# rom1504/clip-retrieval

Hardware: AMD Instinct MI355X
Metric: images/sec embedded (ViT-L/14 bs=256; each sample = image + caption through both towers) (higher is better)
Workload: dtype bf16

## Files before the change

### clip-retrieval_amd/csrc/clip_kernels.hip

```cpp

#include <hip/hip_runtime.h>
#include <stdint.h>
#include <stdlib.h>
#include <math.h>
#include "clip_kernels.h"
#include "gemm_common.h"

namespace clipx {

constexpr int G_TM = 128, G_TN = 128, G_BK = 64;
constexpr int G_STAGE_BYTES = (G_TM + G_TN) * G_BK * 2;
constexpr int G_GROUP_M = 8;

template <int EPI, bool GLDS, bool DEEP = false, bool F16 = false>
__global__ __launch_bounds__(256, (DEEP && !CLIPX_MFMA16) ? 1 : 2) void gemm_bf16_kernel(const bf16* __restrict__ A, const bf16* __restrict__ W,
                                                          const float* __restrict__ bias, void* __restrict__ outp,
                                                          const float* __restrict__ table, int T, int M, int N,
                                                          int K, int row0, const float* __restrict__ rowscale,
                                                          bf16* __restrict__ out16, int kz) {
  extern __shared__ __attribute__((aligned(16))) unsigned char smem[];
  const int tid = threadIdx.x;
  const int lane = tid & 63, w = tid >> 6;
  const int wn = w & 1, wm = w >> 1;
  const int hb = lane >> 5, l31 = lane & 31;
// ... 686 lines not shown
  const dim3 grid((M + 3) / 4), block(256);
#define LN_CASE(NV)                                                                                           \
  case NV * 256:                                                                                              \
    if (out_kind == 1) hipLaunchKernelGGL((layernorm_kernel<NV, 1>), grid, block, 0, st, x, gamma, beta, y, M, eps, (bf16*)nullptr); \
    else if (out_kind == 2) hipLaunchKernelGGL((layernorm_kernel<NV, 2>), grid, block, 0, st, x, gamma, beta, y, M, eps, (bf16*)nullptr); \
    else hipLaunchKernelGGL((layernorm_kernel<NV, 0>), grid, block, 0, st, x, gamma, beta, y, M, eps, y16);    \
    break;
  switch (d) {
    LN_CASE(1) LN_CASE(2) LN_CASE(3) LN_CASE(4) LN_CASE(5) LN_CASE(6) LN_CASE(7) LN_CASE(8)
    default: return hipErrorInvalidValue;
  }
#undef LN_CASE
  return hipGetLastError();
}

template <int FMT>
__global__ __launch_bounds__(256) void im2col_kernel(const void* __restrict__ pixels, int B, int S, int P, int Kp,
                                                    float m0, float m1, float m2, float i0, float i1, float i2,
                                                    bf16* __restrict__ out) {
  const int gdim = S / P, T = gdim * gdim + 1, PP = P * P, K = 3 * PP, nch = Kp / 8;
  const int64_t total = (int64_t)B * T * nch;
  for (int64_t idx = (int64_t)blockIdx.x * blockDim.x + threadIdx.x; idx < total; idx += (int64_t)gridDim.x * blockDim.x) {
    const int ch = (int)(idx % nch);
    const int64_t row = idx / nch;
    const int t = (int)(row % T), b = (int)(row / T);
    bf16x8 o;
    const int tp = t > 0 ? t - 1 : 0;
    const int py = tp / gdim, px = tp - py * gdim;
    float raw[8];
    int cc[8];
#pragma unroll
    for (int e = 0; e < 8; ++e) {
      const int k = ch * 8 + e;
      const int kk = k < K ? k : K - 1;
      const int c = kk / PP, rem = kk - c * PP;
      const int iy = rem / P, ix = rem - iy * P;
      const int yy = py * P + iy, xx = px * P + ix;
      cc[e] = c;
      if (FMT == 0) raw[e] = reinterpret_cast<const float*>(pixels)[(((size_t)b * 3 + c) * S + yy) * S + xx];
      else raw[e] = (float)reinterpret_cast<const unsigned char*>(pixels)[(((size_t)b * S + yy) * S + xx) * 3 + c];
    }
#pragma unroll
    for (int e = 0; e < 8; ++e) {
      float v = raw[e];
      if (FMT != 0) {
        const int c = cc[e];
        const float mean = c == 0 ? m0 : (c == 1 ? m1 : m2), sd = c == 0 ? i0 : (c == 1 ? i1 : i2);
        v = __fdiv_rn(__fsub_rn(__fdiv_rn(v, 255.f), mean), sd);
      }
      o[e] = (t > 0 && ch * 8 + e < K) ? (bf16)v : (bf16)0.f;
    }
    *reinterpret_cast<bf16x8*>(out + (size_t)row * Kp + ch * 8) = o;
  }
}

hipError_t launch_im2col(const void* pixels, int fmt, int B, int S, int P, int Kp, const float* mean,
                         const float* stdv, bf16* out, hipStream_t st) {
  if (B <= 0) return hipSuccess;
  const int gdim = S / P, T = gdim * gdim + 1;
  const int64_t total = (int64_t)B * T * (Kp / 8);
  const int blocks = (int)((total + 255) / 256 < 65536 * 4 ? (total + 255) / 256 : 65536 * 4);
  if (fmt == 0)
    hipLaunchKernelGGL(im2col_kernel<0>, dim3(blocks), dim3(256), 0, st, pixels, B, S, P, Kp, 0.f, 0.f, 0.f, 1.f, 1.f, 1.f, out);
  else
    hipLaunchKernelGGL(im2col_kernel<1>, dim3(blocks), dim3(256), 0, st, pixels, B, S, P, Kp, mean[0], mean[1], mean[2],
                       stdv[0], stdv[1], stdv[2], out);
  return hipGetLastError();
}

__device__ __forceinline__ f32x16 attn_mfma(bf16x8 a, bf16x8 b, f32x16 c) {
  return __builtin_amdgcn_mfma_f32_32x32x16_f16(__builtin_bit_cast(f16x8, a), __builtin_bit_cast(f16x8, b), c, 0, 0, 0);
}
__device__ __forceinline__ unsigned attn_pack_p(float p0, float p1) {
  typedef float f32x2_t __attribute__((ext_vector_type(2)));
  typedef _Float16 f16x2_t __attribute__((ext_vector_type(2)));
  return __builtin_bit_cast(unsigned, __builtin_convertvector((f32x2_t){p0, p1}, f16x2_t));
}

__device__ long long g_attn_phase[8192 * 4];
#ifdef CLIPX_ABLATE
__device__ int g_attn_pk_timer = 0;
#endif
template <int DH, int NKB, int NW, int QPW, bool CAUSAL, bool RECOMP, bool TIMER = false>
__global__ __launch_bounds__(NW * 64, (2 * NW + 3) / 4) void attention_kernel(const bf16* __restrict__ qkv, bf16* __restrict__ out, int Tin,
                                                              int H, float scale_log2e, int dbg, int q_blocks,
                                                              const int* __restrict__ offs, const int* __restrict__ lens) {
  constexpr int TP = NKB * 32;
  constexpr int CH = DH / 8;
  constexpr int KS = DH / 16;
  constexpr int KROW = DH == 64 ? 128 : 176;
  constexpr int DV = (DH + 31) / 32 * 32, NB = DV / 32;
  constexpr int VT_STRIDE = TP * 2 + 8;
  extern __shared__ __attribute__((aligned(16))) unsigned char smem[];
  unsigned char* sK = smem;
  unsigned char* sVt = smem + TP * KROW;
  const int tid = threadIdx.x, lane = tid & 63, w = tid >> 6;
  const int hb = lane >> 5, l31 = lane & 31;
  long long tph[4] = {0, 0, 0, 0};
  long long tst = TIMER ? (long long)__builtin_readcyclecounter() : 0;
#define A_STAMP(i) if (TIMER) { const long long n_ = (long long)__builtin_readcyclecounter(); tph[i] += n_ - tst; tst = n_; }
  const int b = blockIdx.x / H, h = blockIdx.x - b * H;
  const int ld = 3 * H * DH;
  const int T = lens ? lens[b] : Tin;
  const size_t row0 = offs ? (size_t)offs[b] : (size_t)b * Tin;
  const bf16* qbase = qkv + row0 * ld + h * DH;
  const bf16* kbase = qbase + H * DH;
  const bf16* vbase = qbase + 2 * H * DH;
  auto kchunk = [](int key, int c) -> int { return DH == 64 ? (c ^ ((key >> 1) & 7)) : c; };

  bf16x8 qf_all[QPW][KS];
#pragma unroll
  for (int qi = 0; qi < QPW; ++qi) {
    const int qpos = (qi * NW + w) * 32 + l31;
    const int qrow = qpos < T ? qpos : T - 1;
#pragma unroll
    for (int s = 0; s < KS; ++s) {
      const uint4 v = *reinterpret_cast<const uint4*>(qbase + (size_t)qrow * ld + 16 * s + 8 * hb);
      qf_all[qi][s] = *reinterpret_cast<const bf16x8*>(&v);
    }
  }

  if (dbg != 2) {
  {
    constexpr int KIT = (TP * CH + NW * 64 - 1) / (NW * 64);
    uint4 kv[KIT];
#pragma unroll
    for (int it = 0; it < KIT; ++it) {
      const int i = tid + it * NW * 64;
      int key = i / CH;
      const int c = i - key * CH;
      key = key < T ? key : T - 1;
      kv[it] = *reinterpret_cast<const uint4*>(kbase + (size_t)key * ld + c * 8);
    }
#pragma unroll
    for (int it = 0; it < KIT; ++it) {
      const int i = tid + it * NW * 64;
      const int key = i / CH, c = i - key * CH;
      if (i < TP * CH) {
        const uint4 v = key < T ? kv[it] : make_uint4(0u, 0u, 0u, 0u);
        *reinterpret_cast<uint4*>(sK + key * KROW + (kchunk(key, c) << 4)) = v;
      }
    }
  }
  {
    constexpr int VIT = ((TP / 2) * CH + NW * 64 - 1) / (NW * 64);
    uint4 v0s[VIT], v1s[VIT];
#pragma unroll
    for (int it = 0; it < VIT; ++it) {
      const int i = tid + it * NW * 64;
      const int kp = i / CH, c = i - kp * CH;
      const int k0 = 2 * kp < T ? 2 * kp : T - 1, k1 = 2 * kp + 1 < T ? 2 * kp + 1 : T - 1;
      v0s[it] = *reinterpret_cast<const uint4*>(vbase + (size_t)k0 * ld + c * 8);
      v1s[it] = *reinterpret_cast<const uint4*>(vbase + (size_t)k1 * ld + c * 8);
    }
#pragma unroll
    for (int it = 0; it < VIT; ++it) {
      const int i = tid + it * NW * 64;
      const int kp = i / CH, c = i - kp * CH;
      if (i < (TP / 2) * CH) {
        const uint4 v0 = 2 * kp < T ? v0s[it] : make_uint4(0u, 0u, 0u, 0u);
        const uint4 v1 = 2 * kp + 1 < T ? v1s[it] : make_uint4(0u, 0u, 0u, 0u);
        const unsigned a0[4] = {v0.x, v0.y, v0.z, v0.w}, a1[4] = {v1.x, v1.y, v1.z, v1.w};
#pragma unroll
        for (int jj = 0; jj < 4; ++jj) {
          const unsigned lo = (a0[jj] & 0xffffu) | (a1[jj] << 16);
          const unsigned hi = (a0[jj] >> 16) | (a1[jj] & 0xffff0000u);
          *reinterpret_cast<unsigned*>(sVt + (8 * c + 2 * jj) * VT_STRIDE + kp * 4) = lo;
          *reinterpret_cast<unsigned*>(sVt + (8 * c + 2 * jj + 1) * VT_STRIDE + kp * 4) = hi;
        }
      }
    }
    if (DV > DH) {
      for (int i = tid; i < (DV - DH) * (TP / 2); i += NW * 64) {
        const int r = i / (TP / 2), kp = i - r * (TP / 2);
        *reinterpret_cast<unsigned*>(sVt + (DH + r) * VT_STRIDE + kp * 4) = 0u;
      }
    }
  }
  }
  __syncthreads();
  A_STAMP(0)
  if (dbg == 1) return;

  const int ksw = (l31 >> 1) & 7;
#pragma unroll
  for (int qi = 0; qi < QPW; ++qi) {
    const int qb = qi * NW + w;
    if (qb >= q_blocks) break;
    const int qpos = qb * 32 + l31;
    bf16x8 qf[KS];
#pragma unroll
    for (int s = 0; s < KS; ++s) qf[s] = qf_all[qi][s];
    auto s_block = [&](int kb) -> f32x16 {
      f32x16 sb;
#pragma unroll
      for (int r = 0; r < 16; ++r) sb[r] = 0.f;
      if (!CAUSAL || kb <= qb) {
#pragma unroll
        for (int s = 0; s < KS; ++s) {
          const int c = 2 * s + hb;
          const bf16x8 kf = *reinterpret_cast<const bf16x8*>(sK + (kb * 32 + l31) * KROW + ((DH == 64 ? (c ^ ksw) : c) << 4));
          sb = attn_mfma(kf, qf[s], sb);
        }
      }
      if (kb == NKB - 1 || CAUSAL) {
#pragma unroll
        for (int r = 0; r < 16; ++r) {
          const int key = kb * 32 + (r & 3) + 8 * (r >> 2) + 4 * hb;
          const bool ok = key < T && (!CAUSAL || key <= qpos);
          sb[r] = ok ? sb[r] : -INFINITY;
        }
      }
      return sb;
    };
    f32x16 sacc[RECOMP ? 1 : NKB];
    float mx = -INFINITY;
#pragma unroll(RECOMP ? 1 : NKB)
    for (int kb = 0; kb < NKB; ++kb) {
      const f32x16 sb = s_block(kb);
      if (!RECOMP) sacc[kb] = sb;
#pragma unroll
      for (int r = 0; r < 16; ++r) mx = fmaxf(mx, sb[r]);
    }
    mx = fmaxf(mx, __shfl_xor(mx, 32));
    if (mx == -INFINITY) mx = 0.f;
    const float nmx = -mx * scale_log2e;
    if (TIMER) { asm volatile("" : "+v"(mx)); A_STAMP(1) }

    typedef float f32x2_t __attribute__((ext_vector_type(2)));
    typedef __bf16 bf16x2_t __attribute__((ext_vector_type(2)));
    f32x2_t sum2 = {0.f, 0.f};
    const int tail_keys = T - (NKB - 1) * 32;
    f32x16 oacc[NB];
#pragma unroll
    for (int nb = 0; nb < NB; ++nb)
#pragma unroll
      for (int r = 0; r < 16; ++r) oacc[nb][r] = 0.f;
#pragma unroll(RECOMP ? 1 : NKB)
    for (int kb = 0; kb < NKB; ++kb) {
      if (CAUSAL && kb > qb) continue;
      bf16x8 pf[2];
      const f32x16 sb = RECOMP ? s_block(kb) : sacc[RECOMP ? 0 : kb];
      unsigned pw[8];
      const bool short_tail = !CAUSAL && kb == NKB - 1 && tail_keys <= 4;
#pragma unroll
      for (int r = 0; r < 16; r += 2) {
        if (short_tail && r >= 4) {
          pw[r >> 1] = 0u;
          continue;
        }
        const f32x2_t e = (f32x2_t){sb[r], sb[r + 1]} * (f32x2_t){scale_log2e, scale_log2e} + (f32x2_t){nmx, nmx};
        const f32x2_t pp = {__builtin_amdgcn_exp2f(e[0]), __builtin_amdgcn_exp2f(e[1])};
        sum2 += pp;
        pw[r >> 1] = attn_pack_p(pp[0], pp[1]);
      }
      {
        const uint4 w0 = make_uint4(pw[0], pw[1], pw[2], pw[3]), w1 = make_uint4(pw[4], pw[5], pw[6], pw[7]);
        pf[0] = *reinterpret_cast<const bf16x8*>(&w0);
        pf[1] = *reinterpret_cast<const bf16x8*>(&w1);
      }
#pragma unroll
      for (int s2 = 0; s2 < 2; ++s2)
#pragma unroll
        for (int nb = 0; nb < NB; ++nb) {
          const unsigned char* vp = sVt + (32 * nb + l31) * VT_STRIDE + (kb * 32 + 16 * s2 + 4 * hb) * 2;
          const uint2 lo = *reinterpret_cast<const uint2*>(vp);
          const uint2 hi = *reinterpret_cast<const uint2*>(vp + 16);
          uint4 vv = make_uint4(lo.x, lo.y, hi.x, hi.y);
          oacc[nb] = attn_mfma(*reinterpret_cast<bf16x8*>(&vv), pf[s2], oacc[nb]);
        }
    }
    float sum = sum2[0] + sum2[1];
    sum += __shfl_xor(sum, 32);
    const float inv = sum > 0.f ? 1.f / sum : 0.f;
    if (TIMER) { asm volatile("" : "+v"(oacc[0]), "+v"(oacc[NB - 1])); A_STAMP(2) }
    if (qpos < T) {
      bf16* orow = out + (row0 + qpos) * (H * DH) + h * DH;
#pragma unroll
      for (int nb = 0; nb < NB; ++nb)
#pragma unroll
        for (int g = 0; g < 4; ++g) {
          if (32 * nb + 8 * g >= DH) continue;
          bf16x4 o;
#pragma unroll
          for (int e = 0; e < 4; ++e) o[e] = (bf16)(oacc[nb][4 * g + e] * inv);
          *reinterpret_cast<bf16x4*>(orow + 32 * nb + 8 * g + 4 * hb) = o;
        }
    }
    A_STAMP(3)
  }
  if (TIMER && lane == 0 && blockIdx.x * NW + w < 8192) {
#pragma unroll
    for (int i = 0; i < 4; ++i) g_attn_phase[(blockIdx.x * NW + w) * 4 + i] = tph[i];
  }
#undef A_STAMP
}

#ifndef CLIPX_ATTN_SPIPE
#define CLIPX_ATTN_SPIPE 1
#endif
#ifndef CLIPX_ATTN_ROLES
#define CLIPX_ATTN_ROLES 1
#endif
template <int NKB, int NWT = 6>
__global__ __launch_bounds__(NWT * 64, 1) void attention_pk_kernel(const bf16* __restrict__ qkv, bf16* __restrict__ out, int T, int H,
                                                                  int nheads, float scale_log2e, int q_blocks) {
  constexpr bool EIGHT = NWT == 8;
  constexpr int DH = 64, KS = 4, NW = NWT, NDW = EIGHT ? 8 : (CLIPX_ATTN_ROLES ? 2 : 3), QPW = (NKB + NW - 1) / NW, TP = NKB * 32,
                KROW = 128, NB = 2;
  static_assert(NWT == 6 || NWT == 8, "6 waves (any T of NKB blocks) or 8 (T = 32 (NKB - 1) + 1)");
  static_assert(!CLIPX_ATTN_ROLES || NKB == 9, "the role table below is the one of 9 query blocks");
  static_assert(!EIGHT || (NKB == NW + 1 && QPW == 2), "eight full query blocks + the one-query block");
  constexpr int KBYTES = TP * KROW, VHALF = TP * 64, BUF = KBYTES + 2 * VHALF;
  constexpr int KDMA = TP * 8 / 64 / NDW, VDMA = 2 * TP * 4 / 64 / NDW;
  static_assert(EIGHT || TP * 8 % (64 * NDW) == 0, "the DMA pieces must divide evenly among the issuing waves");
  constexpr int NPIECE = BUF / 1024, PPW = NPIECE / 8, KPIECE = KBYTES / 1024;
  static_assert(!EIGHT || NPIECE % 8 == 0, "the DMA pieces must divide evenly among the eight waves");
  constexpr int MRG = 68;
  const bool tail_on = EIGHT && q_blocks >= NKB;
  typedef short s16x4 __attribute__((ext_vector_type(4)));
  typedef s16x4 __attribute__((address_space(3))) * lds_s16x4_ptr;
  extern __shared__ __attribute__((aligned(16))) unsigned char smem[];
  const int tid = threadIdx.x, lane = tid & 63;
  const int w = __builtin_amdgcn_readfirstlane(tid >> 6);
  const int hb = lane >> 5, l31 = lane & 31;
  const int ld = 3 * H * DH;
  const unsigned lds_base = __builtin_amdgcn_readfirstlane((unsigned)(uintptr_t)(__attribute__((address_space(3))) unsigned char*)smem);
#ifdef CLIPX_ABLATE
  const bool timer = g_attn_pk_timer != 0;
  long long tph[4] = {0, 0, 0, 0};
  long long tst = timer ? (long long)__builtin_readcyclecounter() : 0;
#define P_STAMP(i) if (timer) { const long long n_ = (long long)__builtin_readcyclecounter(); tph[i] += n_ - tst; tst = n_; }
#else
#define P_STAMP(i)
#endif

  auto blk_of = [&](int qi) -> int {
    if (EIGHT) return qi == 0 ? w : -1;
#if CLIPX_ATTN_ROLES
    if (qi == 0) return w;
    return w == 0 ? 6 : (w == 2 ? 7 : (w == 3 ? 8 : -1));
#else
    return qi * NW + w < NKB ? qi * NW + w : -1;
#endif
  };
#if CLIPX_ATTN_ROLES
  const bool dma_wave = EIGHT || w == 1 || w == 5;
  const int dma_idx = EIGHT ? w : (w == 1 ? 0 : 1);
#else
  const bool dma_wave = EIGHT || w >= NW - NDW;
  const int dma_idx = EIGHT ? w : w - (NW - NDW);
#endif
  float* mrg = reinterpret_cast<float*>(smem + 2 * BUF);

  auto issue = [&](int hd, int buf) {
    if (!dma_wave) return;
    const int ww = dma_idx;
    const int b = hd / H, h = hd - b * H;
    const char* base = reinterpret_cast<const char*>(qkv + (size_t)b * T * ld + h * DH);
    int lane_v = lane;
    asm volatile("" : "+v"(lane_v));
    if constexpr (EIGHT) {
#pragma unroll
      for (int j = 0; j < PPW; ++j) {
        const int piece = ww * PPW + j;
        unsigned off;
        if (piece < KPIECE) {
          const int c = piece * 64 + lane_v;
          const int key = c >> 3, pos = c & 7;
          const int kk = key < T ? key : T - 1;
          off = (unsigned)((kk * ld + H * DH + ((pos ^ ((key >> 1) & 7)) << 3)) * 2);
        } else {
          const int c = (piece - KPIECE) * 64 + lane_v;
          const int nbh = c / (TP * 4), rem = c - nbh * (TP * 4);
          const int key = rem >> 2, pos = rem & 3;
          const int kk = key < T ? key : T - 1;
          off = (unsigned)((kk * ld + 2 * H * DH + 32 * nbh + 8 * pos) * 2);
        }
        const unsigned m0 = lds_base + buf * BUF + piece * 1024;
        asm volatile("s_mov_b32 m0, %2\n\ts_nop 0\n\tglobal_load_lds_dwordx4 %0, %1" ::"v"(off), "s"(base), "s"(m0) : "memory");
      }
      return;
    }
#pragma unroll
    for (int j = 0; j < KDMA; ++j) {
      const int c = (ww * KDMA + j) * 64 + lane_v;
      const int key = c >> 3, pos = c & 7;
      const int kk = key < T ? key : T - 1;
      const unsigned off = (unsigned)((kk * ld + H * DH + ((pos ^ ((key >> 1) & 7)) << 3)) * 2);
      const unsigned m0 = lds_base + buf * BUF + (ww * KDMA + j) * 1024;
      asm volatile("s_mov_b32 m0, %2\n\ts_nop 0\n\tglobal_load_lds_dwordx4 %0, %1" ::"v"(off), "s"(base), "s"(m0) : "memory");
    }
#pragma unroll
    for (int j = 0; j < VDMA; ++j) {
      const int c = (ww * VDMA + j) * 64 + lane_v;
      const int nbh = c / (TP * 4), rem = c - nbh * (TP * 4);
      const int key = rem >> 2, pos = rem & 3;
      const int kk = key < T ? key : T - 1;
      const unsigned off = (unsigned)((kk * ld + 2 * H * DH + 32 * nbh + 8 * pos) * 2);
      const unsigned m0 = lds_base + buf * BUF + KBYTES + (ww * VDMA + j) * 1024;
      asm volatile("s_mov_b32 m0, %2\n\ts_nop 0\n\tglobal_load_lds_dwordx4 %0, %1" ::"v"(off), "s"(base), "s"(m0) : "memory");
    }
  };
  bf16x8 qn[QPW][KS];
  auto load_q = [&](int hd, int qi) {
    const int b = hd / H, h = hd - b * H;
    const bf16* qbase = qkv + (size_t)b * T * ld + h * DH;
    int lane_q = lane;
    asm volatile("" : "+v"(lane_q));
    if (blk_of(qi) < 0) return;
    const int qpos = blk_of(qi) * 32 + (lane_q & 31);
    const int qrow = qpos < T ? qpos : T - 1;
#pragma unroll
    for (int s = 0; s < KS; ++s) {
      const uint4 v = *reinterpret_cast<const uint4*>(qbase + (size_t)qrow * ld + 16 * s + 8 * (lane_q >> 5));
      qn[qi][s] = *reinterpret_cast<const bf16x8*>(&v);
    }
  };

  bf16x8 qt[KS];
  auto load_qt = [&](int hd) {
    const int b = hd / H, h = hd - b * H;
    const bf16* qbase = qkv + (size_t)b * T * ld + h * DH;
    int lane_q = lane;
    asm volatile("" : "+v"(lane_q));
#pragma unroll
    for (int s = 0; s < KS; ++s) {
      const uint4 v = *reinterpret_cast<const uint4*>(qbase + (size_t)(T - 1) * ld + 16 * s + 8 * (lane_q >> 5));
      qt[s] = *reinterpret_cast<const bf16x8*>(&v);
    }
  };
  auto merge_tail = [&](int phd, int par) {
    const float* mt = mrg + par * (NKB * MRG);
    float m = -INFINITY;
#pragma unroll
    for (int j = 0; j < NKB; ++j) m = fmaxf(m, mt[j * MRG]);
    float l = 0.f, o = 0.f;
#pragma unroll
    for (int j = 0; j < NKB; ++j) {
      const float wj = __builtin_amdgcn_exp2f((mt[j * MRG] - m) * scale_log2e);
      l += wj * mt[j * MRG + 1];
      o += wj * mt[j * MRG + 2 + lane];
    }
    const int pb = phd / H, ph = phd - pb * H;
    out[((size_t)pb * T + (T - 1)) * (H * DH) + ph * DH + lane] = (bf16)(l > 0.f ? o / l : 0.f);
  };

  int hd = blockIdx.x;
  if (hd >= nheads) return;
  issue(hd, 0);
#pragma unroll
  for (int qi = 0; qi < QPW; ++qi) load_q(hd, qi);
  if (tail_on) {
    load_qt(hd);
#pragma unroll
    for (int s = 0; s < KS; ++s) asm volatile("" : "+v"(qt[s]));
  }
#pragma unroll
  for (int qi = 0; qi < QPW; ++qi)
#pragma unroll
    for (int s = 0; s < KS; ++s) asm volatile("" : "+v"(qn[qi][s]));
  const int ksw = (l31 >> 1) & 7;
  const unsigned vlane = (unsigned)(((lane & 15) >> 2) * 64 + (16 * ((lane >> 4) & 1)) * 2 + (lane & 3) * 8);
  int buf = 0;
  for (; hd < nheads; hd += gridDim.x, buf ^= 1) {
    if (dma_wave && !(hd != (int)blockIdx.x && w < q_blocks)) asm volatile("s_waitcnt vmcnt(0)" ::: "memory");
    __syncthreads();
    P_STAMP(0)
    const int nxt = hd + gridDim.x;
    if (nxt < nheads) issue(nxt, buf ^ 1);
    P_STAMP(1)
    if (tail_on && w == 0 && hd != (int)blockIdx.x) merge_tail(hd - (int)gridDim.x, buf ^ 1);
    const unsigned char* sK = smem + buf * BUF;
    const unsigned char* sV = sK + KBYTES;
    const int b = hd / H, h = hd - b * H;
#pragma unroll
    for (int qi = 0; qi < QPW; ++qi) {
      const int qb = blk_of(qi);
      if (qb < 0 || qb >= q_blocks) continue;
      const int qpos = qb * 32 + l31;
      bf16x8 qf[KS];
#pragma unroll
      for (int s = 0; s < KS; ++s) qf[s] = qn[qi][s];
      f32x16 sacc[NKB];
      float mx = -INFINITY;
#if CLIPX_ATTN_SPIPE
      {
        typedef int i32x4 __attribute__((ext_vector_type(4)));
        unsigned kaddr[KS];
#pragma unroll
        for (int s = 0; s < KS; ++s) kaddr[s] = lds_base + buf * BUF + l31 * KROW + (((2 * s + hb) ^ ksw) << 4);
        i32x4 KF[2][KS];
#pragma unroll
        for (int s = 0; s < KS; ++s) asm volatile("ds_read_b128 %0, %1" : "=v"(KF[0][s]) : "v"(kaddr[s]));
        __builtin_amdgcn_sched_barrier(0);
#pragma unroll
        for (int kb = 0; kb < NKB; ++kb) {
          asm volatile("s_waitcnt lgkmcnt(0)" ::: "memory");
#pragma unroll
          for (int s = 0; s < KS; ++s) asm volatile("" : "+v"(KF[kb & 1][s]));
          if (kb + 1 < NKB) {
#pragma unroll
            for (int s = 0; s < KS; ++s)
              asm volatile("ds_read_b128 %0, %1 offset:%2" : "=v"(KF[(kb + 1) & 1][s]) : "v"(kaddr[s]), "n"((kb + 1) * 32 * KROW));
          }
          __builtin_amdgcn_sched_barrier(0);
          f32x16 sb;
#pragma unroll
          for (int r = 0; r < 16; ++r) sb[r] = 0.f;
#pragma unroll
          for (int s = 0; s < KS; ++s) sb = attn_mfma(__builtin_bit_cast(bf16x8, KF[kb & 1][s]), qf[s], sb);
          __builtin_amdgcn_sched_barrier(0);
          if (kb > 0) {
#pragma unroll
            for (int r = 0; r < 16; ++r) mx = fmaxf(mx, sacc[kb - 1][r]);
            asm volatile("" : "+v"(mx));
            __builtin_amdgcn_sched_barrier(0);
          }
          if (kb == NKB - 1) {
#pragma unroll
            for (int r = 0; r < 16; ++r) {
              const int key = kb * 32 + (r & 3) + 8 * (r >> 2) + 4 * hb;
              sb[r] = key < T ? sb[r] : -INFINITY;
            }
          }
          sacc[kb] = sb;
        }
#pragma unroll
        for (int r = 0; r < 16; ++r) mx = fmaxf(mx, sacc[NKB - 1][r]);
      }
#else
#pragma unroll
      for (int kb = 0; kb < NKB; ++kb) {
        f32x16 sb;
#pragma unroll
        for (int r = 0; r < 16; ++r) sb[r] = 0.f;
#pragma unroll
        for (int s = 0; s < KS; ++s) {
          const int c = 2 * s + hb;
          const bf16x8 kf = *reinterpret_cast<const bf16x8*>(sK + (kb * 32 + l31) * KROW + ((c ^ ksw) << 4));
          sb = attn_mfma(kf, qf[s], sb);
        }
        if (kb == NKB - 1) {
#pragma unroll
          for (int r = 0; r < 16; ++r) {
            const int key = kb * 32 + (r & 3) + 8 * (r >> 2) + 4 * hb;
            sb[r] = key < T ? sb[r] : -INFINITY;
          }
        }
        sacc[kb] = sb;
#pragma unroll
        for (int r = 0; r < 16; ++r) mx = fmaxf(mx, sb[r]);
      }
#endif
#ifdef CLIPX_ABLATE
      if (timer) { asm volatile("" : "+v"(mx)); P_STAMP(2) }
#endif
#if !CLIPX_ATTN_SPIPE
      if (nxt < nheads) load_q(nxt, qi);
#endif
      mx = fmaxf(mx, __shfl_xor(mx, 32));
      if (mx == -INFINITY) mx = 0.f;
      const float nmx = -mx * scale_log2e;
      typedef float f32x2_t __attribute__((ext_vector_type(2)));
      typedef __bf16 bf16x2_t __attribute__((ext_vector_type(2)));
      f32x2_t sum2 = {0.f, 0.f};
      const int tail_keys = T - (NKB - 1) * 32;
      f32x16 oacc[NB];
#pragma unroll
      for (int nb = 0; nb < NB; ++nb)
#pragma unroll
        for (int r = 0; r < 16; ++r) oacc[nb][r] = 0.f;
#if CLIPX_ATTN_SPIPE
      {
        typedef short s16x8 __attribute__((ext_vector_type(8)));
        unsigned pw[8];
        unsigned pnew[8];
        s16x8 vf[2][NB];
        auto read_v = [&](int kb, int s2) {
#pragma unroll
          for (int nb = 0; nb < NB; ++nb) {
            const unsigned char* vp = sV + nb * VHALF + (kb * 32 + 16 * s2 + 4 * hb) * 64 + vlane;
            const s16x4 lo = __builtin_amdgcn_ds_read_tr16_b64_v4i16((lds_s16x4_ptr)(vp));
            const s16x4 hi = __builtin_amdgcn_ds_read_tr16_b64_v4i16((lds_s16x4_ptr)(vp + 8 * 64));
            vf[s2][nb] = __builtin_shufflevector(lo, hi, 0, 1, 2, 3, 4, 5, 6, 7);
          }
        };
        auto p_chunk = [&](int kb, int c, unsigned* dst) {
          const bool short_tail = kb == NKB - 1 && tail_keys <= 4;
          float nmx_c = nmx;
          asm volatile("" : "+v"(nmx_c));
#pragma unroll
          for (int r = 4 * c; r < 4 * c + 4; r += 2) {
            if (short_tail && r >= 4) {
              dst[r >> 1] = 0u;
              continue;
            }
            const f32x2_t e = (f32x2_t){sacc[kb][r], sacc[kb][r + 1]} * (f32x2_t){scale_log2e, scale_log2e} + (f32x2_t){nmx_c, nmx_c};
            const f32x2_t pp = {__builtin_amdgcn_exp2f(e[0]), __builtin_amdgcn_exp2f(e[1])};
            sum2 += pp;
            dst[r >> 1] = attn_pack_p(pp[0], pp[1]);
          }
          asm volatile("" : "+v"(dst[2 * c]), "+v"(dst[2 * c + 1]));
        };
        auto pv_mfma = [&](int m) {
          const int s2 = m >> 1, nb = m & 1;
          const uint4 w4 = make_uint4(pw[4 * s2], pw[4 * s2 + 1], pw[4 * s2 + 2], pw[4 * s2 + 3]);
          oacc[nb] = attn_mfma(__builtin_bit_cast(bf16x8, vf[s2][nb]), *reinterpret_cast<const bf16x8*>(&w4), oacc[nb]);
        };
        read_v(0, 0);
#pragma unroll
        for (int c = 0; c < 4; ++c) p_chunk(0, c, pw);
        __builtin_amdgcn_sched_barrier(0);
#pragma unroll
        for (int kb = 1; kb < NKB; ++kb) {
          pv_mfma(0);
          __builtin_amdgcn_sched_barrier(0);
          p_chunk(kb, 0, pnew);
          __builtin_amdgcn_sched_barrier(0);
          pv_mfma(1);
          __builtin_amdgcn_sched_barrier(0);
          read_v(kb - 1, 1);
          p_chunk(kb, 1, pnew);
          __builtin_amdgcn_sched_barrier(0);
          pv_mfma(2);
          __builtin_amdgcn_sched_barrier(0);
          p_chunk(kb, 2, pnew);
          __builtin_amdgcn_sched_barrier(0);
          pv_mfma(3);
          __builtin_amdgcn_sched_barrier(0);
          read_v(kb, 0);
          p_chunk(kb, 3, pnew);
#pragma unroll
          for (int e = 0; e < 8; ++e) pw[e] = pnew[e];
          if (kb == NKB / 2 && nxt < nheads) load_q(nxt, qi);
          __builtin_amdgcn_sched_barrier(0);
        }
        pv_mfma(0);
        pv_mfma(1);
        read_v(NKB - 1, 1);
        pv_mfma(2);
        pv_mfma(3);
      }
#else
#pragma unroll
      for (int kb = 0; kb < NKB; ++kb) {
        bf16x8 pf[2];
        const f32x16 sb = sacc[kb];
        unsigned pw[8];
        const bool short_tail = kb == NKB - 1 && tail_keys <= 4;
#pragma unroll
        for (int r = 0; r < 16; r += 2) {
          if (short_tail && r >= 4) {
            pw[r >> 1] = 0u;
            continue;
          }
          const f32x2_t e = (f32x2_t){sb[r], sb[r + 1]} * (f32x2_t){scale_log2e, scale_log2e} + (f32x2_t){nmx, nmx};
          const f32x2_t pp = {__builtin_amdgcn_exp2f(e[0]), __builtin_amdgcn_exp2f(e[1])};
          sum2 += pp;
          pw[r >> 1] = attn_pack_p(pp[0], pp[1]);
        }
        {
          const uint4 w0 = make_uint4(pw[0], pw[1], pw[2], pw[3]), w1 = make_uint4(pw[4], pw[5], pw[6], pw[7]);
          pf[0] = *reinterpret_cast<const bf16x8*>(&w0);
          pf[1] = *reinterpret_cast<const bf16x8*>(&w1);
        }
#pragma unroll
        for (int s2 = 0; s2 < 2; ++s2)
#pragma unroll
          for (int nb = 0; nb < NB; ++nb) {
            const unsigned char* vp = sV + nb * VHALF + (kb * 32 + 16 * s2 + 4 * hb) * 64 + vlane;
            const s16x4 lo = __builtin_amdgcn_ds_read_tr16_b64_v4i16((lds_s16x4_ptr)(vp));
            const s16x4 hi = __builtin_amdgcn_ds_read_tr16_b64_v4i16((lds_s16x4_ptr)(vp + 8 * 64));
            typedef short s16x8 __attribute__((ext_vector_type(8)));
            const s16x8 vv = __builtin_shufflevector(lo, hi, 0, 1, 2, 3, 4, 5, 6, 7);
            oacc[nb] = attn_mfma(__builtin_bit_cast(bf16x8, vv), pf[s2], oacc[nb]);
          }
      }
#endif
      float sum = sum2[0] + sum2[1];
      sum += __shfl_xor(sum, 32);
      const float inv = sum > 0.f ? 1.f / sum : 0.f;
#pragma unroll
      for (int s = 0; s < KS; ++s) asm volatile("" : "+v"(qn[qi][s]));
      if (tail_on) {
#pragma unroll
        for (int s = 0; s < KS; ++s) asm volatile("" : "+v"(qt[s]));
      }
      if (dma_wave) asm volatile("s_waitcnt vmcnt(0)" ::: "memory");
      int lane_o = lane;
      asm volatile("" : "+v"(lane_o));
      const int opos = qb * 32 + (lane_o & 31);
      if (opos < T) {
        bf16* orow = out + ((size_t)b * T + opos) * (H * DH) + h * DH;
#pragma unroll
        for (int nb = 0; nb < NB; ++nb)
#pragma unroll
          for (int g = 0; g < 4; ++g) {
            bf16x4 o;
#pragma unroll
            for (int e = 0; e < 4; ++e) o[e] = (bf16)(oacc[nb][4 * g + e] * inv);
            *reinterpret_cast<bf16x4*>(orow + 32 * nb + 8 * g + 4 * (lane_o >> 5)) = o;
          }
      }
      P_STAMP(3)
    }
    if (tail_on) {
      bf16x8 qtl[KS];
#pragma unroll
      for (int s = 0; s < KS; ++s) qtl[s] = qt[s];
#pragma unroll
      for (int rep = 0; rep < 2; ++rep) {
        if (rep == 1 && w != 0) break;
        const int kb = rep == 0 ? w : NKB - 1;
        f32x16 sb;
#pragma unroll
        for (int r = 0; r < 16; ++r) sb[r] = 0.f;
#pragma unroll
        for (int s = 0; s < KS; ++s) {
          const int c = 2 * s + hb;
          const bf16x8 kf = *reinterpret_cast<const bf16x8*>(sK + (kb * 32 + l31) * KROW + ((c ^ ksw) << 4));
          sb = attn_mfma(kf, qtl[s], sb);
        }
        if (rep == 0 && nxt < nheads && w != 0) load_qt(nxt);
        if (rep == 1 && nxt < nheads) load_qt(nxt);
        if (kb == NKB - 1) {
#pragma unroll
          for (int r = 0; r < 16; ++r) {
            const int key = kb * 32 + (r & 3) + 8 * (r >> 2) + 4 * hb;
            sb[r] = key < T ? sb[r] : -INFINITY;
          }
        }
        float mx = -INFINITY;
#pragma unroll
        for (int r = 0; r < 16; ++r) mx = fmaxf(mx, sb[r]);
        mx = fmaxf(mx, __shfl_xor(mx, 32));
        const float nmx = -mx * scale_log2e;
        typedef float f32x2_t __attribute__((ext_vector_type(2)));
        f32x2_t sum2 = {0.f, 0.f};
        unsigned pw[8];
        const bool first_quad_only = kb == NKB - 1 && T - (NKB - 1) * 32 <= 4;
#pragma unroll
        for (int r = 0; r < 16; r += 2) {
          if (first_quad_only && r >= 4) {
            pw[r >> 1] = 0u;
            continue;
          }
          const f32x2_t e = (f32x2_t){sb[r], sb[r + 1]} * (f32x2_t){scale_log2e, scale_log2e} + (f32x2_t){nmx, nmx};
          const f32x2_t pp = {__builtin_amdgcn_exp2f(e[0]), __builtin_amdgcn_exp2f(e[1])};
          sum2 += pp;
          pw[r >> 1] = attn_pack_p(pp[0], pp[1]);
        }
        f32x16 oacc[NB];
#pragma unroll
        for (int nb = 0; nb < NB; ++nb)
#pragma unroll
          for (int r = 0; r < 16; ++r) oacc[nb][r] = 0.f;
#pragma unroll
        for (int s2 = 0; s2 < 2; ++s2) {
          const uint4 w4 = make_uint4(pw[4 * s2], pw[4 * s2 + 1], pw[4 * s2 + 2], pw[4 * s2 + 3]);
#pragma unroll
          for (int nb = 0; nb < NB; ++nb) {
            const unsigned char* vp = sV + nb * VHALF + (kb * 32 + 16 * s2 + 4 * hb) * 64 + vlane;
            const s16x4 lo = __builtin_amdgcn_ds_read_tr16_b64_v4i16((lds_s16x4_ptr)(vp));
            const s16x4 hi = __builtin_amdgcn_ds_read_tr16_b64_v4i16((lds_s16x4_ptr)(vp + 8 * 64));
            typedef short s16x8 __attribute__((ext_vector_type(8)));
            const s16x8 vv = __builtin_shufflevector(lo, hi, 0, 1, 2, 3, 4, 5, 6, 7);
            oacc[nb] = attn_mfma(__builtin_bit_cast(bf16x8, vv), *reinterpret_cast<const bf16x8*>(&w4), oacc[nb]);
          }
        }
        float sum = sum2[0] + sum2[1];
        sum += __shfl_xor(sum, 32);
        if (l31 == 0) {
          float* m = mrg + buf * (NKB * MRG) + kb * MRG;
          if (hb == 0) {
            m[0] = mx;
            m[1] = sum;
          }
#pragma unroll
          for (int nb = 0; nb < NB; ++nb)
#pragma unroll
            for (int g = 0; g < 4; ++g)
#pragma unroll
              for (int e = 0; e < 4; ++e) m[2 + 32 * nb + 8 * g + 4 * hb + e] = oacc[nb][4 * g + e];
        }
      }
    }
  }
  if (tail_on) {
    __syncthreads();
    if (w == 0) merge_tail(hd - (int)gridDim.x, buf ^ 1);
  }
#ifdef CLIPX_ABLATE
  if (timer && lane == 0 && blockIdx.x * NW + w < 8192) {
#pragma unroll
    for (int i = 0; i < 4; ++i) g_attn_phase[(blockIdx.x * NW + w) * 4 + i] = tph[i];
  }
#endif
#undef P_STAMP
}

static int attn_cu_count() {
  static int n = 0;
  if (n == 0) {
    int dev = 0, v = 0;
    if (hipGetDevice(&dev) == hipSuccess && hipDeviceGetAttribute(&v, hipDeviceAttributeMultiprocessorCount, dev) == hipSuccess && v > 0) n = v;
    else n = 256;
  }
  return n;
}

static hipError_t launch_attention_pk9(const bf16* qkv, bf16* out, int B, int T, int H, hipStream_t st, int q_blocks) {
  constexpr int NKB = 9, TP = NKB * 32;
  const size_t smem = (size_t)2 * (TP * 128 + 2 * TP * 64);
  const int nheads = B * H, grid = std::min(nheads, attn_cu_count());
#ifdef CLIPX_ABLATE
  static const int cfg8 = getenv("CLIPX_ATTN_CFG") ? atoi(getenv("CLIPX_ATTN_CFG")) : 0;
  if (cfg8 == 13 && T == (NKB - 1) * 32 + 1) {
    const size_t smem8 = smem + (size_t)2 * NKB * 68 * sizeof(float);
    auto k8 = attention_pk_kernel<NKB, 8>;
    hipError_t e8 = hipFuncSetAttribute(reinterpret_cast<const void*>(k8), hipFuncAttributeMaxDynamicSharedMemorySize, (int)smem8);
    if (e8 != hipSuccess) return e8;
    hipLaunchKernelGGL(k8, dim3(grid), dim3(512), smem8, st, qkv, out, T, H, nheads, (1.f / 8.f) * 1.4426950408889634f,
                       q_blocks > 0 && q_blocks < NKB ? q_blocks : NKB);
    return hipGetLastError();
  }
#endif
  auto kern = attention_pk_kernel<NKB>;
  hipError_t e = hipFuncSetAttribute(reinterpret_cast<const void*>(kern), hipFuncAttributeMaxDynamicSharedMemorySize, (int)smem);
  if (e != hipSuccess) return e;
#ifdef CLIPX_ABLATE
  static const int qb_env = getenv("CLIPX_ATTN_QBLOCKS") ? atoi(getenv("CLIPX_ATTN_QBLOCKS")) : 0;
  if (qb_env > 0) q_blocks = qb_env;
  static const int timer_env = getenv("CLIPX_ATTN_PK_TIMER") ? atoi(getenv("CLIPX_ATTN_PK_TIMER")) : 0;
  static bool timer_set = false;
  if (!timer_set) {
    timer_set = true;
    (void)hipMemcpyToSymbol(HIP_SYMBOL(g_attn_pk_timer), &timer_env, sizeof(int));
  }
#endif
  hipLaunchKernelGGL(kern, dim3(grid), dim3(384), smem, st, qkv, out, T, H, nheads, (1.f / 8.f) * 1.4426950408889634f,
                     q_blocks > 0 && q_blocks < NKB ? q_blocks : NKB);
  return hipGetLastError();
}

#ifdef CLIPX_ABLATE
extern "C" int clipx_dbg_attn_phase(long long* host, int n) {
  return (int)hipMemcpyFromSymbol(host, HIP_SYMBOL(g_attn_phase), (size_t)n * sizeof(long long));
}
#endif

template <int DH, int NKB, int NW, int QPW, bool RECOMP = false>
static hipError_t launch_attention_cfg(const bf16* qkv, bf16* out, int B, int T, int H, int causal, hipStream_t st, int q_blocks,
                                       const int* offs = nullptr, const int* lens = nullptr) {
  q_blocks = q_blocks > 0 && q_blocks < NKB ? q_blocks : NKB;
  constexpr int KROW = DH == 64 ? 128 : 176, DV = (DH + 31) / 32 * 32;
  const size_t smem = (size_t)NKB * 32 * KROW + (size_t)DV * (NKB * 64 + 8);
  const float scale_log2e = (1.f / sqrtf((float)DH)) * 1.4426950408889634f;
  const dim3 grid(B * H), block(NW * 64);
#ifdef CLIPX_ABLATE
  static const int dbg = getenv("CLIPX_ATTN_DBG") ? atoi(getenv("CLIPX_ATTN_DBG")) : 0;
#else
  constexpr int dbg = 0;
#endif
  if (causal) {
    auto kern = attention_kernel<DH, NKB, NW, QPW, true, RECOMP>;
    hipError_t e = hipFuncSetAttribute(reinterpret_cast<const void*>(kern), hipFuncAttributeMaxDynamicSharedMemorySize, (int)smem);
    if (e != hipSuccess) return e;
    hipLaunchKernelGGL(kern, grid, block, smem, st, qkv, out, T, H, scale_log2e, dbg, q_blocks, offs, lens);
  } else {
    auto kern = attention_kernel<DH, NKB, NW, QPW, false, RECOMP>;
    hipError_t e = hipFuncSetAttribute(reinterpret_cast<const void*>(kern), hipFuncAttributeMaxDynamicSharedMemorySize, (int)smem);
    if (e != hipSuccess) return e;
    hipLaunchKernelGGL(kern, grid, block, smem, st, qkv, out, T, H, scale_log2e, dbg, q_blocks, offs, lens);
  }
  return hipGetLastError();
}

hipError_t launch_attention(const bf16* qkv, bf16* out, int B, int T, int H, int dh, int causal, hipStream_t st, int q_blocks,
                            const int* offs, const int* lens) {
  if (B <= 0) return hipSuccess;
  if ((offs != nullptr) != (lens != nullptr)) return hipErrorInvalidValue;
  if (offs && (dh != 64 || (T + 31) / 32 > 4)) return hipErrorInvalidValue;
  const int nkb = (T + 31) / 32;
  if (dh == 80) {
    switch (nkb) {
      case 1: return launch_attention_cfg<80, 1, 1, 1>(qkv, out, B, T, H, causal, st, q_blocks);
      case 2: return launch_attention_cfg<80, 2, 2, 1>(qkv, out, B, T, H, causal, st, q_blocks);
      case 3: return launch_attention_cfg<80, 3, 3, 1>(qkv, out, B, T, H, causal, st, q_blocks);
      case 9: return launch_attention_cfg<80, 9, 9, 1, true>(qkv, out, B, T, H, causal, st, q_blocks);
      default: return hipErrorInvalidValue;
    }
  }
  if (dh != 64) return hipErrorInvalidValue;
  switch (nkb) {
    case 1: return launch_attention_cfg<64, 1, 1, 1>(qkv, out, B, T, H, causal, st, q_blocks, offs, lens);
    case 2: return launch_attention_cfg<64, 2, 2, 1>(qkv, out, B, T, H, causal, st, q_blocks, offs, lens);
    case 3: return launch_attention_cfg<64, 3, 3, 1>(qkv, out, B, T, H, causal, st, q_blocks, offs, lens);
    case 4: return launch_attention_cfg<64, 4, 4, 1>(qkv, out, B, T, H, causal, st, q_blocks, offs, lens);
    case 5: return launch_attention_cfg<64, 5, 3, 2>(qkv, out, B, T, H, causal, st, q_blocks);
    case 6: return launch_attention_cfg<64, 6, 3, 2>(qkv, out, B, T, H, causal, st, q_blocks);
    case 7: return launch_attention_cfg<64, 7, 4, 2>(qkv, out, B, T, H, causal, st, q_blocks);
    case 8: return launch_attention_cfg<64, 8, 4, 2>(qkv, out, B, T, H, causal, st, q_blocks);
    case 9: {
#ifdef CLIPX_ABLATE
      static const int cfg = getenv("CLIPX_ATTN_CFG") ? atoi(getenv("CLIPX_ATTN_CFG")) : 0;
#else
      constexpr int cfg = 0;
#endif
      if (cfg == 4) return launch_attention_cfg<64, 9, 4, 3>(qkv, out, B, T, H, causal, st, q_blocks);
#ifdef CLIPX_ABLATE
      if (cfg == 5) return launch_attention_cfg<64, 9, 9, 1, true>(qkv, out, B, T, H, causal, st, q_blocks);
      if (cfg == 6) return launch_attention_cfg<64, 9, 5, 2>(qkv, out, B, T, H, causal, st, q_blocks);
      if (cfg == 7) return launch_attention_cfg<64, 9, 9, 1>(qkv, out, B, T, H, causal, st, q_blocks);
      if (cfg == 8) return launch_attention_cfg<64, 9, 5, 2, true>(qkv, out, B, T, H, causal, st, q_blocks);
#endif
      if (cfg == 9 && !causal) {
        constexpr int KROW = 128, DV = 64;
        const size_t smem = (size_t)9 * 32 * KROW + (size_t)DV * (9 * 64 + 8);
        auto kern = attention_kernel<64, 9, 3, 3, false, false, true>;
        hipError_t e = hipFuncSetAttribute(reinterpret_cast<const void*>(kern), hipFuncAttributeMaxDynamicSharedMemorySize, (int)smem);
        if (e != hipSuccess) return e;
        hipLaunchKernelGGL(kern, dim3(B * H), dim3(192), smem, st, qkv, out, T, H, (1.f / 8.f) * 1.4426950408889634f, 0, 9, (const int*)nullptr, (const int*)nullptr);
        return hipGetLastError();
      }
#ifdef CLIPX_ABLATE
      if (cfg == 10 || causal) return launch_attention_cfg<64, 9, 3, 3>(qkv, out, B, T, H, causal, st, q_blocks);
#else
      if (causal) return launch_attention_cfg<64, 9, 3, 3>(qkv, out, B, T, H, causal, st, q_blocks);
#endif
      return launch_attention_pk9(qkv, out, B, T, H, st, q_blocks);
    }
    default: return hipErrorInvalidValue;
  }
}

__global__ __launch_bounds__(256) void text_embed_kernel(const int32_t* __restrict__ ids, const float* __restrict__ tok,
                                                        const float* __restrict__ pos, float* __restrict__ x, int BT,
                                                        int T, int d, int vocab, void* __restrict__ x16, int x16_f16,
                                                        const int* __restrict__ rowmap) {
  const int d4 = d / 4;
  const int64_t total = (int64_t)BT * d4;
  for (int64_t idx = (int64_t)blockIdx.x * blockDim.x + threadIdx.x; idx < total; idx += (int64_t)gridDim.x * blockDim.x) {
    const int c = (int)(idx % d4);
    const int row = (int)(idx / d4);
    const int src = rowmap ? rowmap[row] : row;
    int id = ids[src];
    id = id < 0 ? 0 : (id >= vocab ? vocab - 1 : id);
    const float4 a = reinterpret_cast<const float4*>(tok + (size_t)id * d)[c];
    const float4 p = reinterpret_cast<const float4*>(pos + (size_t)(src % T) * d)[c];
    const float4 o = make_float4(a.x + p.x, a.y + p.y, a.z + p.z, a.w + p.w);
    if (x) reinterpret_cast<float4*>(x + (size_t)row * d)[c] = o;
    if (x16 && x16_f16) {
      f16x4 h;
      h[0] = (_Float16)o.x; h[1] = (_Float16)o.y; h[2] = (_Float16)o.z; h[3] = (_Float16)o.w;
      reinterpret_cast<f16x4*>(reinterpret_cast<_Float16*>(x16) + (size_t)row * d)[c] = h;
    } else if (x16) {
      bf16x4 h;
      h[0] = (bf16)o.x; h[1] = (bf16)o.y; h[2] = (bf16)o.z; h[3] = (bf16)o.w;
      reinterpret_cast<bf16x4*>(reinterpret_cast<bf16*>(x16) + (size_t)row * d)[c] = h;
    }
  }
}

hipError_t launch_text_embed(const int32_t* ids, const float* tok_emb, const float* pos_emb, float* x, int B, int T, int d,
                             int vocab, hipStream_t st, void* x16, int x16_f16, const int* rowmap, int nrows) {
  if (B <= 0) return hipSuccess;
  const int rows = rowmap ? nrows : B * T;
  if (rows <= 0) return hipSuccess;
  const int64_t total = (int64_t)rows * (d / 4);
  const int blocks = (int)((total + 255) / 256);
  hipLaunchKernelGGL(text_embed_kernel, dim3(blocks), dim3(256), 0, st, ids, tok_emb, pos_emb, x, rows, T, d, vocab, x16, x16_f16, rowmap);
  return hipGetLastError();
}

__device__ __forceinline__ float block_sum_256(float v, float* red) {
  for (int o = 32; o > 0; o >>= 1) v += __shfl_xor(v, o);
  __syncthreads();
  if ((threadIdx.x & 63) == 0) red[threadIdx.x >> 6] = v;
  __syncthreads();
  return red[0] + red[1] + red[2] + red[3];
}

__global__ __launch_bounds__(256) void tail_proj_kernel(const void* __restrict__ x, const int32_t* __restrict__ ids,
                                                       const float* __restrict__ gamma, const float* __restrict__ beta,
                                                       const bf16* __restrict__ proj, float* __restrict__ o_raw, int T, int d,
                                                       int E, float eps, int x_f16, int* __restrict__ range_flag) {
  extern __shared__ __attribute__((aligned(16))) unsigned char smem[];
  float* y = reinterpret_cast<float*>(smem);
  float* red = y + d;
  int* s_posp = reinterpret_cast<int*>(red + 4);
  const int b = blockIdx.y, tid = threadIdx.x;
// ... 130 lines not shown
```

Baseline: 5978.

## Add trickle K/V DMA and pad-skip options; hand-schedule softmax exp chunk

```diff
diff --git a/clip-retrieval_amd/csrc/clip_kernels.hip b/clip-retrieval_amd/csrc/clip_kernels.hip
--- a/clip-retrieval_amd/csrc/clip_kernels.hip
+++ b/clip-retrieval_amd/csrc/clip_kernels.hip
@@ -1012,6 +1012,12 @@
 #ifndef CLIPX_ATTN_ROLES
 #define CLIPX_ATTN_ROLES 1
 #endif
+#ifndef CLIPX_ATTN_SKIP_PAD
+#define CLIPX_ATTN_SKIP_PAD 0
+#endif
+#ifndef CLIPX_ATTN_TRICKLE
+#define CLIPX_ATTN_TRICKLE 0
+#endif
 template <int NKB, int NWT = 6>
 __global__ __launch_bounds__(NWT * 64, 1) void attention_pk_kernel(const bf16* __restrict__ qkv, bf16* __restrict__ out, int T, int H,
                                                                   int nheads, float scale_log2e, int q_blocks) {
@@ -1062,6 +1068,11 @@
   const int dma_idx = EIGHT ? w : w - (NW - NDW);
 #endif
   float* mrg = reinterpret_cast<float*>(smem + 2 * BUF);
+  constexpr bool TRICKLE = CLIPX_ATTN_TRICKLE && CLIPX_ATTN_ROLES && CLIPX_ATTN_SPIPE && !EIGHT;
+  constexpr bool SKIP_PAD = CLIPX_ATTN_SKIP_PAD && !EIGHT;
+  constexpr int VPI = TP / 16;
+  static_assert(!TRICKLE || (NPIECE == 4 * NKB * 2 && KPIECE == NPIECE / 2), "two waves x two blocks x NKB key blocks x two pieces");
+  static_assert(!TRICKLE || NPIECE % NW == 0, "the first pair's pieces are dealt evenly over the waves");
 
   auto issue = [&](int hd, int buf) {
     if (!dma_wave) return;
@@ -1094,6 +1105,7 @@
     }
 #pragma unroll
     for (int j = 0; j < KDMA; ++j) {
+      if (SKIP_PAD && (ww * KDMA + j) * 8 >= T) continue;
       const int c = (ww * KDMA + j) * 64 + lane_v;
       const int key = c >> 3, pos = c & 7;
       const int kk = key < T ? key : T - 1;
@@ -1103,6 +1115,7 @@
     }
 #pragma unroll
     for (int j = 0; j < VDMA; ++j) {
+      if (SKIP_PAD && ((ww * VDMA + j) % VPI) * 16 >= T) continue;
       const int c = (ww * VDMA + j) * 64 + lane_v;
       const int nbh = c / (TP * 4), rem = c - nbh * (TP * 4);
       const int key = rem >> 2, pos = rem & 3;
@@ -1112,6 +1125,46 @@
       asm volatile("s_mov_b32 m0, %2\n\ts_nop 0\n\tglobal_load_lds_dwordx4 %0, %1" ::"v"(off), "s"(base), "s"(m0) : "memory");
     }
   };
+  auto issue_pieces = [&](const char* base, int buf, int p0, int n) {
+    int lane_v = lane;
+    asm volatile("" : "+v"(lane_v));
+#pragma unroll 1
+    for (int piece = p0; piece < p0 + n; ++piece) {
+      unsigned off;
+      if (piece < KPIECE) {
+        if (SKIP_PAD && piece * 8 >= T) continue;
+        const int c = piece * 64 + lane_v;
+        const int key = c >> 3, pos = c & 7;
+        const int kk = key < T ? key : T - 1;
+        off = (unsigned)((kk * ld + H * DH + ((pos ^ ((key >> 1) & 7)) << 3)) * 2);
+      } else {
+        const int v = piece - KPIECE;
+        if (SKIP_PAD && (v % VPI) * 16 >= T) continue;
+        const int nbh = v / VPI, rem = (v % VPI) * 64 + lane_v;
+        const int key = rem >> 2, pos = rem & 3;
+        const int kk = key < T ? key : T - 1;
+        off = (unsigned)((kk * ld + 2 * H * DH + 32 * nbh + 8 * pos) * 2);
+      }
+      const unsigned m0 = lds_base + buf * BUF + piece * 1024;
+      asm volatile("s_mov_b32 m0, %2\n\ts_nop 0\n\tglobal_load_lds_dwordx4 %0, %1" ::"v"(off), "s"(base), "s"(m0) : "memory");
+    }
+  };
+  auto pair_base = [&](int hd) -> const char* {
+    const int b = hd / H, h = hd - b * H;
+    return reinterpret_cast<const char*>(qkv + (size_t)b * T * ld + h * DH);
+  };
+  const bool tr_s = TRICKLE && q_blocks >= NKB;
+#if CLIPX_ATTN_TRICKLE == 2
+  constexpr int TRN = 1;
+  const bool tr_wave = tr_s && w != 5;
+  const int tr_p0 = w == 0 ? 0 : (w == 1 ? 2 * NKB : (w == 2 ? 3 * NKB : (w == 3 ? 5 * NKB : 7 * NKB)));
+  static_assert(!TRICKLE || NPIECE == 8 * NKB, "waves 0, 2, 3: 2 NKB slots each, waves 1, 4: NKB each");
+#else
+  constexpr int TRN = 2;
+  const bool tr_wave = tr_s && (w == 2 || w == 3);
+  const int tr_p0 = w == 2 ? 0 : KPIECE;
+#endif
+  constexpr int BURST = (NPIECE + NW - 2) / (NW - 1);
   bf16x8 qn[QPW][KS];
   auto load_q = [&](int hd, int qi) {
     const int b = hd / H, h = hd - b * H;
@@ -1158,7 +1211,20 @@
 
   int hd = blockIdx.x;
   if (hd >= nheads) return;
-  issue(hd, 0);
+  if (SKIP_PAD) {
+    const int k0 = (T + 7) & ~7, v0 = (T + 15) & ~15;
+#pragma unroll
+    for (int half = 0; half < 2; ++half) {
+      unsigned char* img = smem + half * BUF;
+      for (int i = k0 * KROW + tid * 16; i < TP * KROW; i += NW * 64 * 16) *reinterpret_cast<uint4*>(img + i) = make_uint4(0, 0, 0, 0);
+#pragma unroll
+      for (int nb = 0; nb < NB; ++nb)
+        for (int i = v0 * 64 + tid * 16; i < TP * 64; i += NW * 64 * 16)
+          *reinterpret_cast<uint4*>(img + KBYTES + nb * VHALF + i) = make_uint4(0, 0, 0, 0);
+    }
+  }
+  if (TRICKLE) issue_pieces(pair_base(hd), 0, w * (NPIECE / NW), NPIECE / NW);
+  else issue(hd, 0);
 #pragma unroll
   for (int qi = 0; qi < QPW; ++qi) load_q(hd, qi);
   if (tail_on) {
@@ -1174,11 +1240,18 @@
   const unsigned vlane = (unsigned)(((lane & 15) >> 2) * 64 + (16 * ((lane >> 4) & 1)) * 2 + (lane & 3) * 8);
   int buf = 0;
   for (; hd < nheads; hd += gridDim.x, buf ^= 1) {
-    if (dma_wave && !(hd != (int)blockIdx.x && w < q_blocks)) asm volatile("s_waitcnt vmcnt(0)" ::: "memory");
+    if (TRICKLE ? (hd == (int)blockIdx.x || (!tr_s && w >= 1)) : (dma_wave && !(hd != (int)blockIdx.x && w < q_blocks)))
+      asm volatile("s_waitcnt vmcnt(0)" ::: "memory");
     __syncthreads();
     P_STAMP(0)
     const int nxt = hd + gridDim.x;
-    if (nxt < nheads) issue(nxt, buf ^ 1);
+    const char* nbase = nullptr;
+    if (TRICKLE) {
+      if (nxt < nheads) {
+        nbase = pair_base(nxt);
+        if (!tr_s && w >= 1) issue_pieces(nbase, buf ^ 1, (w - 1) * BURST, w == NW - 1 ? NPIECE - (NW - 2) * BURST : BURST);
+      }
+    } else if (nxt < nheads) issue(nxt, buf ^ 1);
     P_STAMP(1)
     if (tail_on && w == 0 && hd != (int)blockIdx.x) merge_tail(hd - (int)gridDim.x, buf ^ 1);
     const unsigned char* sK = smem + buf * BUF;
@@ -1225,6 +1298,10 @@
 #pragma unroll
             for (int r = 0; r < 16; ++r) mx = fmaxf(mx, sacc[kb - 1][r]);
             asm volatile("" : "+v"(mx));
+            __builtin_amdgcn_sched_barrier(0);
+          }
+          if (TRICKLE && tr_wave && nbase != nullptr) {
+            issue_pieces(nbase, buf ^ 1, tr_p0 + (qi * NKB + kb) * TRN, TRN);
             __builtin_amdgcn_sched_barrier(0);
           }
           if (kb == NKB - 1) {
@@ -1287,6 +1364,7 @@
         unsigned pw[8];
         unsigned pnew[8];
         s16x8 vf[2][NB];
+        float sum_e = 0.f, sum_o = 0.f;
         auto read_v = [&](int kb, int s2) {
 #pragma unroll
           for (int nb = 0; nb < NB; ++nb) {
@@ -1298,20 +1376,30 @@
         };
         auto p_chunk = [&](int kb, int c, unsigned* dst) {
           const bool short_tail = kb == NKB - 1 && tail_keys <= 4;
-          float nmx_c = nmx;
-          asm volatile("" : "+v"(nmx_c));
-#pragma unroll
-          for (int r = 4 * c; r < 4 * c + 4; r += 2) {
-            if (short_tail && r >= 4) {
-              dst[r >> 1] = 0u;
-              continue;
-            }
-            const f32x2_t e = (f32x2_t){sacc[kb][r], sacc[kb][r + 1]} * (f32x2_t){scale_log2e, scale_log2e} + (f32x2_t){nmx_c, nmx_c};
-            const f32x2_t pp = {__builtin_amdgcn_exp2f(e[0]), __builtin_amdgcn_exp2f(e[1])};
-            sum2 += pp;
-            dst[r >> 1] = attn_pack_p(pp[0], pp[1]);
+          if (short_tail && c >= 1) {
+            dst[2 * c] = 0u;
+            dst[2 * c + 1] = 0u;
+            asm volatile("" : "+v"(dst[2 * c]), "+v"(dst[2 * c + 1]));
+            return;
           }
-          asm volatile("" : "+v"(dst[2 * c]), "+v"(dst[2 * c + 1]));
+          float e0, e1, e2, e3;
+          asm volatile(
+              "v_fma_f32 %2, %8, %9, %13\n\t"
+              "v_fma_f32 %3, %8, %10, %13\n\t"
+              "v_fma_f32 %4, %8, %11, %13\n\t"
+              "v_fma_f32 %5, %8, %12, %13\n\t"
+              "v_exp_f32 %2, %2\n\t"
+              "v_exp_f32 %3, %3\n\t"
+              "v_exp_f32 %4, %4\n\t"
+              "v_exp_f32 %5, %5\n\t"
+              "v_add_f32 %6, %6, %2\n\t"
+              "v_add_f32 %7, %7, %3\n\t"
+              "v_cvt_pk_f16_f32 %0, %2, %3\n\t"
+              "v_add_f32 %6, %6, %4\n\t"
+              "v_add_f32 %7, %7, %5\n\t"
+              "v_cvt_pk_f16_f32 %1, %4, %5"
+              : "=v"(dst[2 * c]), "=v"(dst[2 * c + 1]), "=&v"(e0), "=&v"(e1), "=&v"(e2), "=&v"(e3), "+v"(sum_e), "+v"(sum_o)
+              : "s"(scale_log2e), "v"(sacc[kb][4 * c]), "v"(sacc[kb][4 * c + 1]), "v"(sacc[kb][4 * c + 2]), "v"(sacc[kb][4 * c + 3]), "v"(nmx));
         };
         auto pv_mfma = [&](int m) {
           const int s2 = m >> 1, nb = m & 1;
@@ -1351,6 +1439,7 @@
         read_v(NKB - 1, 1);
         pv_mfma(2);
         pv_mfma(3);
+        sum2 = (f32x2_t){sum_e, sum_o};
       }
 #else
 #pragma unroll
@@ -1397,7 +1486,7 @@
 #pragma unroll
         for (int s = 0; s < KS; ++s) asm volatile("" : "+v"(qt[s]));
       }
-      if (dma_wave) asm volatile("s_waitcnt vmcnt(0)" ::: "memory");
+      if (TRICKLE ? tr_wave : dma_wave) asm volatile("s_waitcnt vmcnt(0)" ::: "memory");
       int lane_o = lane;
       asm volatile("" : "+v"(lane_o));
       const int opos = qb * 32 + (lane_o & 31);
```

Measured after the change: 5977. No clear change (-0.0%).
